# neu-vi/Superpoints_Registration

Measured on AMD Instinct MI355X. Metric: point-cloud pairs/sec (16 384 pts/cloud), higher is better.
Workload: dtype f32 (matrix products: range-scaled split-f16x2 MFMA, f32 accumulate; attention weights below 2^-5 of their row sum carried in one f16 plane); 1 GPU; synthetic 16384-pt pairs, full KPConv backbone + superpoint attn + Sinkhorn-SVD pose (3dmatch config, BASELINE configs[1]); streams_per_gpu=1, points_per_cloud=16384, generator=box, point_order=reference, upsample_indices=True, cross_step_overlap=True, streams_inside_a_forward=3: main path, pyramid searches, ResNet shortcut branches

## Files before the change

### include/spr.h

```cpp
#ifndef SPR_H_
#define SPR_H_

#include <stddef.h>
#include <stdint.h>

#ifdef __cplusplus
extern "C" {
#endif

#define SPR_VERSION 6

#define SPR_ACT_NONE 0
#define SPR_ACT_RELU 1
#define SPR_ACT_SIGMOID 2

#define SPR_ORDER_REFERENCE 0
#define SPR_ORDER_CANONICAL 1

#define SPR_SELECT_NEAREST 0
#define SPR_SELECT_INDEX 1

int spr_version(void);
const char* spr_last_error(void);

// ... 75 lines not shown
                      int k, unsigned int* rkeys, unsigned int* extra, float* noise, unsigned int* skeys, void* stream);
size_t spr_modelnet_pairs_workspace_size(int n_total, int nb, int k);
int spr_modelnet_pairs(const float* xyz, const int* cu, int n_total, int nb, int max_len_host, float p_src, float p_tgt,
                       double q_src, double q_tgt, int k, float scale, float clip, const float* transform,
                       const double* dirs, uint64_t seed, const uint64_t* pair_key, const unsigned int* rkeys,
                       const unsigned int* extra, const float* noise, const unsigned int* skeys, float* src_xyz,
                       float* tgt_xyz, float* pose, unsigned char* src_overlap, unsigned char* tgt_overlap,
                       int* src_index, int* tgt_index, int* corr, int* corr_count, int* status, void* ws,
                       size_t ws_bytes, void* stream);

size_t spr_kpconv_workspace_bytes(int nq, int ns, int cin, int cout);
size_t spr_kpconv_plan_bytes(int nq);
int spr_kpconv_plan(const int* nbr, int nq, int ns, int nbr_stride, int kmax, int rows_sorted,
                    const int* order, void* plan, size_t plan_bytes, void* stream);
size_t spr_kpconv_wplanes_bytes(int cin, int cout);
int spr_kpconv_prep_weights(const float* weights, int n_kp, int cin, int cout, const float* w_range,
                            int w_range_n, void* wplanes, size_t wplanes_bytes, void* stream);
int spr_kpconv_fwd(const float* q_xyz, int nq, const float* s_xyz, int ns, const int* nbr,
                   int nbr_stride, int kmax, int rows_sorted, const float* x, int cin,
                   const float* weights, int cout, const float* kernel_points, int n_kp,
                   float kp_extent, float* out, int impl, const float* x_range, int x_range_n,
                   const float* w_range, int w_range_n, const void* plan, const void* wplanes,
                   void* ws, size_t ws_bytes, void* stream);

size_t spr_instnorm_workspace_bytes(int max_len_host, int nb, int c);
int spr_instnorm(const float* x, const int* cu, int n, int nb, int max_len_host, int c,
                 float eps, int norm, const float* add, float slope, float* out,
                 float* out_range, int out_range_n, void* ws, size_t ws_bytes, void* stream);
int spr_instnorm_stats(const float* x, const int* cu, int n, int nb, int max_len_host, int c, float eps,
                       float* mean, float* rstd, void* ws, size_t ws_bytes, void* stream);

int spr_block_tail_tile_rows(int ka, int kb, int n_out);
size_t spr_block_tail_tiles_len(int n, int nb, int tile_rows);
int spr_block_tail_tiles(const int* cu, int n, int nb, int tile_rows, int* tiles, void* stream);
size_t spr_block_tail_workspace_bytes(int n, int nb, int kb, int n_out, int tile_rows);
int spr_block_tail(const float* xa, int ka, const float* wa, const float* xb, int kb, const float* wb,
                   const float* add, const int* cu, const int* tiles, int n, int nb, int n_out, float eps,
                   float slope, float* out, const float* xa_range, int xa_range_n, const float* wa_range,
                   int wa_range_n, const float* xb_range, int xb_range_n, const float* wb_range,
                   int wb_range_n, float* out_range, int out_range_n, const float* xa_mean,
                   const float* xa_rstd, float xa_slope, void* ws, size_t ws_bytes, void* stream);

int spr_maxpool_gather(const float* x, int ns, int c, const int* idx, int nq, int idx_stride, int k,
                       const int* order, float* out, float* out_range, int out_range_n, void* stream);
size_t spr_cell_order_workspace_bytes(int n);
int spr_cell_order(const float* xyz, const int* cu, int n, int nb, float cell, int* order, void* ws, size_t ws_bytes,
// ... 242 lines not shown
```

### superpoints_registration_amd/_lib.py

```python
import ctypes
import os
import subprocess

_HERE = os.path.dirname(os.path.abspath(__file__))
LIB_PATH = os.environ.get("SPR_HIP_LIB") or os.path.join(_HERE, "libspr_hip.so")

_vp = ctypes.c_void_p
_i = ctypes.c_int
_f = ctypes.c_float
_sz = ctypes.c_size_t
_l = ctypes.c_long
_u64 = ctypes.c_uint64
_d = ctypes.c_double

SIGNATURES = {
    "spr_version": (_i, []),
    "spr_last_error": (ctypes.c_char_p, []),
    "spr_grid_subsample_workspace_bytes": (_sz, [_i, _i]),
    "spr_grid_subsample": (_i, [_vp, _vp, _i, _i, _f, _i, _i, _vp, _vp, _vp, _vp, _sz, _vp]),
    "spr_voxel_downsample_workspace_bytes": (_sz, [_i]),
    "spr_voxel_downsample": (_i, [_vp, _i, ctypes.c_double, _vp, _vp, _vp, _sz, _vp]),
    "spr_prepare_scans_scratch_len": (_sz, [_i, _i]),
    "spr_prepare_scans": (_i, [_vp, _i, _vp, _i, _i, ctypes.c_double, ctypes.c_double, _i, _vp, _sz, _vp, _vp, _vp, _vp,
                               _vp]),
# ... 8 lines not shown
    "spr_radius_table_count": (_i, [_vp, _vp, _i, _i, _i, _i, _f, _vp, _vp, _vp, _i, _vp, _vp]),
    "spr_kdtree_replay_size": (_sz, [_i, _i]),
    "spr_kdtree_replay_build": (_i, [_vp, _vp, _i, _i, _vp, _sz, _vp]),
    "spr_tie_order_workspace_size": (_sz, [_i, _i, _i]),
    "spr_tie_order": (_i, [_vp, _vp, _i, _vp, _vp, _i, _i, _f, _vp, _i, _vp, _i, _i, _i, _vp, _vp, _sz, _vp]),
    "spr_tie_order_host": (_i, [_vp, _vp, _i, _vp, _vp, _i, _i, _f, _vp, _i, _i, _i, _vp]),
    "spr_std_sort_replay_host": (_i, [_vp, _i, _vp, _vp]),
    "spr_gt_overlap_workspace_bytes": (_sz, [_i, _i, _i]),
    "spr_gt_overlap": (_i, [_vp, _vp, _i, _vp, _vp, _i, _vp, _i, ctypes.c_double, _vp, _vp, _vp, _vp, _vp, _vp, _vp,
                            _sz, _vp]),
    "spr_philox4x32_host": (_i, [_vp, _vp, _vp]),
    "spr_augment_draw": (_i, [_u64, _vp, _i, _i, _vp, _vp, _vp, _vp, _vp, _i, _vp, _i, _vp, _vp, _vp]),
    "spr_augment_workspace_bytes": (_sz, [_i, _i, _i, _i]),
    "spr_augment_pairs": (_i, [_vp, _vp, _i, _vp, _vp, _i, _vp, _i, _vp, _vp, _vp, _i, _vp, _vp, _vp, _vp, _i, _f, _i,
                               _u64, _vp, _vp, _vp, _vp, _vp, _vp, _vp, _vp, _vp, _vp, _vp, _vp, _vp, _vp, _vp, _vp,
                               _sz, _vp]),
    "spr_modelnet_draw": (_i, [_u64, _vp, _i, _d, _d, _vp, _vp, _vp, _vp, _i, _i, _vp, _vp, _vp, _vp, _vp]),
    "spr_modelnet_pairs_workspace_size": (_sz, [_i, _i, _i]),
    "spr_modelnet_pairs": (_i, [_vp, _vp, _i, _i, _i, _f, _f, _d, _d, _i, _f, _f, _vp, _vp, _u64, _vp, _vp, _vp, _vp,
                                _vp, _vp, _vp, _vp, _vp, _vp, _vp, _vp, _vp, _vp, _vp, _vp, _sz, _vp]),
    "spr_kpconv_workspace_bytes": (_sz, [_i, _i, _i, _i]),
    "spr_kpconv_fwd": (_i, [_vp, _i, _vp, _i, _vp, _i, _i, _i, _vp, _i, _vp, _i, _vp, _i, _f, _vp, _i, _vp, _i, _vp,
                            _i, _vp, _vp, _vp, _sz, _vp]),
    "spr_instnorm_workspace_bytes": (_sz, [_i, _i, _i]),
    "spr_instnorm": (_i, [_vp, _vp, _i, _i, _i, _i, _f, _i, _vp, _f, _vp, _vp, _i, _vp, _sz, _vp]),
    "spr_maxpool_gather": (_i, [_vp, _i, _i, _vp, _i, _i, _i, _vp, _vp, _vp, _i, _vp]),
    "spr_linear_workspace_bytes": (_sz, []),
    "spr_linear": (_i, [_vp, _i, _i, _vp, _i, _vp, _vp, _i, _vp, _vp, _i, _vp, _i, _vp, _i, _vp, _vp, _sz, _vp]),
    "spr_range_parts": (_i, []),
    "spr_absmax_multi": (_i, [_vp, _i, _i, _vp, _vp]),
    "spr_absmax": (_i, [_vp, _l, _i, _l, _vp, _vp]),
    "spr_kpconv_plan_bytes": (_sz, [_i]),
    "spr_kpconv_plan": (_i, [_vp, _i, _i, _i, _i, _i, _vp, _vp, _sz, _vp]),
    "spr_kpconv_wplanes_bytes": (_sz, [_i, _i]),
    "spr_kpconv_prep_weights": (_i, [_vp, _i, _i, _i, _vp, _i, _vp, _sz, _vp]),
    "spr_block_tail_tile_rows": (_i, [_i, _i, _i]),
    "spr_block_tail_tiles_len": (_sz, [_i, _i, _i]),
    "spr_block_tail_tiles": (_i, [_vp, _i, _i, _i, _vp, _vp]),
    "spr_block_tail_workspace_bytes": (_sz, [_i, _i, _i, _i, _i]),
    "spr_block_tail": (_i, [_vp, _i, _vp, _vp, _i, _vp, _vp, _vp, _vp, _i, _i, _i, _f, _f, _vp, _vp, _i, _vp, _i,
                            _vp, _i, _vp, _i, _vp, _i, _vp, _vp, _f, _vp, _sz, _vp]),
    "spr_instnorm_stats": (_i, [_vp, _vp, _i, _i, _i, _i, _f, _vp, _vp, _vp, _sz, _vp]),
    "spr_cell_order_workspace_bytes": (_sz, [_i]),
    "spr_cell_order": (_i, [_vp, _vp, _i, _i, _f, _vp, _vp, _sz, _vp]),
    "spr_layernorm_range_count": (_i, [_i]),
    "spr_attn_inproj_prepare": (_i, [_vp, _i, _vp, _vp]),
# ... 124 lines not shown
```

### superpoints_registration_amd/csrc/kpconv.hip

```cpp
#include "lds_dma.h"
#include "spr_common.h"
#include "split_mma.h"

namespace spr {
namespace {

constexpr int kKP = 15;

__global__ __launch_bounds__(256) void k_rowflag(const float* __restrict__ x, const float* __restrict__ s_xyz,
                                                 int ns, int cin, unsigned char* __restrict__ flag,
                                                 float4* __restrict__ sxf, int* __restrict__ tile_ctr) {
  const int wid = (blockIdx.x * blockDim.x + threadIdx.x) >> 6;
  const int lane = threadIdx.x & 63;
  const int c4 = cin >> 2;
  if (blockIdx.x == 0 && threadIdx.x == 0) {
    sxf[ns] = make_float4(-1.0e17f, -1.0e17f, -1.0e17f, __int_as_float(0));
    tile_ctr[0] = 0;
  }
  if ((cin & 3) == 0 && c4 <= 64 && (c4 & (c4 - 1)) == 0) {
    constexpr int kRfSteps = 4;
    const int rpl = 64 / c4;
    const int sub = lane / c4, chunk = lane % c4;
    const int row0 = wid * rpl * kRfSteps + sub;
    float4 v[kRfSteps];
// ... 64 lines not shown
    cnt += flag[idx];
    const float rx = s_xyz[3 * (size_t)idx] - qx, ry = s_xyz[3 * (size_t)idx + 1] - qy,
                rz = s_xyz[3 * (size_t)idx + 2] - qz;
    for (int p = 0; p < n_kp; ++p) {
      const float dx = rx - kpts[3 * p], dy = ry - kpts[3 * p + 1], dz = rz - kpts[3 * p + 2];
      const float w = fmaxf(0.f, 1.f - sqrtf(dx * dx + dy * dy + dz * dz) * inv_extent);
      if (w > 0.f) {
        float d = 0.f;
        for (int c = 0; c < cin; ++c)
          d += x[(size_t)idx * cin + c] * W[((size_t)p * cin + c) * cout + o];
        acc += w * d;
      }
    }
  }
  out[(size_t)n * cout + o] = acc / (float)max(cnt, 1);
}

__global__ __launch_bounds__(256) void k_records_cin1(const float* __restrict__ x, const float* __restrict__ s_xyz,
                                                      int ns, float4* __restrict__ sxf) {
  const int i = blockIdx.x * blockDim.x + threadIdx.x;
  if (i < ns) sxf[i] = make_float4(s_xyz[3 * (size_t)i], s_xyz[3 * (size_t)i + 1], s_xyz[3 * (size_t)i + 2], x[i]);
}

__global__ __launch_bounds__(256) void k_kpconv_cin1(
    const float* __restrict__ q_xyz, int nq, const float* __restrict__ s_xyz, int ns,
    const int* __restrict__ nbr, int nbr_stride, int kmax, int rows_sorted,
    const float4* __restrict__ sxf, const float* __restrict__ W, int cout,
    const float* __restrict__ kpts, int n_kp, float inv_extent, float* __restrict__ out) {
  const int lane = threadIdx.x & 63, wave = threadIdx.x >> 6;
  const int qv = lane & 15, g = lane >> 4;
  const int q0 = blockIdx.x * 64 + wave * 16;
  if (q0 >= nq) return;
  const int n = min(q0 + qv, nq - 1);
  const float qx = q_xyz[3 * (size_t)n], qy = q_xyz[3 * (size_t)n + 1], qz = q_xyz[3 * (size_t)n + 2];
  float kx[4], ky[4], kz[4];
  bool kok[4];
#pragma unroll
  for (int s = 0; s < 4; ++s) {
    const int p = 4 * s + g;
    kok[s] = p < n_kp;
    kx[s] = kok[s] ? kpts[3 * p] : 0.f;
    ky[s] = kok[s] ? kpts[3 * p + 1] : 0.f;
    kz[s] = kok[s] ? kpts[3 * p + 2] : 0.f;
  }
  float wf[4] = {0.f, 0.f, 0.f, 0.f};
  int cnt = 0;
  const int* row = nbr + (size_t)n * nbr_stride;
  for (int k = 0; k < kmax; ++k) {
    const int idx = row[k];
    const bool ok = idx >= 0 && idx < ns;
    if (rows_sorted && __ballot(ok) == 0ull) break;
    const size_t id = ok ? (size_t)idx : 0;
    const float4 rec = sxf[id];
    const float xv = ok ? rec.w : 0.f;
    cnt += xv > 0.f ? 1 : 0;
    const float rx = rec.x - qx, ry = rec.y - qy, rz = rec.z - qz;
#pragma unroll
    for (int s = 0; s < 4; ++s) {
      const float dx = rx - kx[s], dy = ry - ky[s], dz = rz - kz[s];
      const float w = fmaxf(0.f, 1.f - __builtin_amdgcn_sqrtf(dx * dx + dy * dy + dz * dz) * inv_extent);
      wf[s] += kok[s] ? w * xv : 0.f;
    }
  }
  const float inv = 1.f / (float)max(cnt, 1);
#pragma unroll
  for (int s = 0; s < 4; ++s) wf[s] *= inv;
  for (int o0 = 0; o0 < cout; o0 += 16) {
    f32x4 acc = {0.f, 0.f, 0.f, 0.f};
#pragma unroll
    for (int s = 0; s < 4; ++s) {
      const int p = 4 * s + g;
      const float bv = (p < n_kp && o0 + qv < cout) ? W[(size_t)p * cout + o0 + qv] : 0.f;
      acc = __builtin_amdgcn_mfma_f32_16x16x4f32(wf[s], bv, acc, 0, 0, 0);
    }
#pragma unroll
    for (int r = 0; r < 4; ++r) {
      const int qn = q0 + 4 * g + r;
      if (qn < nq && o0 + qv < cout) out[(size_t)qn * cout + o0 + qv] = acc[r];
    }
  }
}

__global__ __launch_bounds__(256) void k_w_prep(const float* __restrict__ W, int cin, int cout, int cc,
                                                const float* __restrict__ w_parts, int n_wparts,
                                                _Float16* __restrict__ Wh, _Float16* __restrict__ Wl) {
  __shared__ float sh[17];
  const float sb = pow2f(pow2_exp_for(block_absmax(w_parts, sh, n_wparts)));
  const int total = kKP * cin * cout;
  const int i = blockIdx.x * blockDim.x + threadIdx.x;
  if (i >= total) return;
  const int KS = kKP * cc / 32, NT = cout / 16;
  const int e = i & 7, lane = (i >> 3) & 63;
  int r = i >> 9;
  const int ks = r % KS;
  r /= KS;
  const int nt = r % NT, chunk = r / NT;
  const int p16 = lane & 15, j4 = lane >> 4;
  const int kk = 32 * ks + 8 * j4 + e;
  const int p = kk / cc, c = chunk * cc + kk % cc;
  const float w = W[((size_t)p * cin + c) * cout + 16 * nt + p16] * sb;
  const _Float16 h = (_Float16)w;
  Wh[i] = h;
  Wl[i] = (_Float16)(w - (float)h);
// ... 843 lines not shown
extern "C" size_t spr_kpconv_wplanes_bytes(int cin, int cout) {
  return measure(wplanes_view, cin, cout);
}

extern "C" int spr_kpconv_prep_weights(const float* weights, int n_kp, int cin, int cout, const float* w_range,
                                       int w_range_n, void* wplanes, size_t bytes, void* stream_) {
  hipStream_t stream = (hipStream_t)stream_;
  SPR_REQUIRE(n_kp == kKP && cin % 32 == 0 && cout % 32 == 0 && cout <= 256,
              "kpconv weight planes exist for the MFMA shapes only (15 kernel points, channels in multiples of 32)");
  SPR_REQUIRE(w_range != nullptr && w_range_n >= 1, "kpconv weight planes: the weight range is required");
  Workspace w(wplanes, bytes);
  const auto [wh, wl] = wplanes_view(w, cin, cout);
  SPR_REQUIRE(wplanes != nullptr && w.ok(), "kpconv weight planes: buffer too small");
  hipLaunchKernelGGL(k_w_prep, dim3(cdiv((long)n_kp * cin * cout, 256)), dim3(256), 0, stream, weights, cin, cout,
                     w_chunk(cin), w_range, w_range_n, wh, wl);
  SPR_LAUNCH_CHECK();
  return 0;
}

extern "C" size_t spr_kpconv_workspace_bytes(int nq, int ns, int cin, int cout) {
  return measure(kpconv_layout, nq, ns, cin, cout);
}

extern "C" int spr_kpconv_fwd(const float* q_xyz, int nq, const float* s_xyz, int ns,
                              const int* nbr, int nbr_stride, int kmax, int rows_sorted,
                              const float* x, int cin, const float* weights, int cout,
                              const float* kernel_points, int n_kp, float kp_extent,
                              float* out, int impl, const float* x_range, int x_range_n, const float* w_range,
                              int w_range_n, const void* plan, const void* wplanes, void* ws, size_t ws_bytes,
                              void* stream_) {
  hipStream_t stream = (hipStream_t)stream_;
  SPR_REQUIRE((x_range == nullptr || x_range_n >= 1) && (w_range == nullptr || w_range_n >= 1),
              "kpconv: a range needs a count");
  SPR_REQUIRE(nq > 0 && ns > 0, "kpconv: empty input");
  SPR_REQUIRE(kmax >= 1 && kmax <= nbr_stride, "kpconv: bad kmax=%d stride=%d", kmax, nbr_stride);
  SPR_REQUIRE(cin >= 1 && cout >= 1 && n_kp >= 1 && n_kp <= 32, "kpconv: bad dims");
  SPR_REQUIRE(kp_extent > 0.f, "kpconv: KP_extent must be > 0");
  Workspace w(ws, ws_bytes);
  const auto [flag, sxf, own_wplanes, x_parts, w_parts, own_plan, tile_ctr] = kpconv_layout(w, nq, ns, cin, cout);
  SPR_REQUIRE(ws != nullptr && w.ok(), "kpconv: workspace too small");
  SPR_REQUIRE(wplanes == nullptr || w_range != nullptr, "kpconv: prepared weight planes come with the range they were scaled by");
  Workspace given_w(const_cast<void*>(wplanes), SIZE_MAX), given_p(const_cast<void*>(plan), SIZE_MAX);
  const auto [wh, wl] = wplanes != nullptr ? wplanes_view(given_w, cin, cout) : own_wplanes;
  const float inv_extent = 1.0f / kp_extent;

  if (cin == 1 && (impl == 0 || impl == 2) && n_kp <= 16) {
// ... 66 lines not shown
```

### superpoints_registration_amd/csrc/linear.hip

```cpp
#include <atomic>

#include "attn_planes.h"
#include "lds_dma.h"
#include "spr_common.h"
#include "split_mma.h"

namespace spr {
namespace {

constexpr int BK = 32;
static_assert(BK == kPlaneK, "the split kernels stage split_mma.h's slabs");
constexpr int LDSK = BK + 1;

template <int ACT, bool RES>
__device__ __forceinline__ float store_tile(const f32x16& acc, int row0, int col, int M, int N,
                                            float bv, const float* __restrict__ residual,
                                            float* __restrict__ out, int lh, float unscale = 1.0f,
                                            const float* __restrict__ epi = nullptr) {
  if (col >= N) return 0.f;
  float vmax = 0.f;
  float res[16];
  if (RES) {
#pragma unroll
    for (int r = 0; r < 16; ++r) {
// ... 588 lines not shown
      *reinterpret_cast<float4*>(out_pos + o) = yp;
    }
  }
  if (range_norm || range_pos) {
    mxn = wave_max(mxn);
    mxp = wave_max(mxp);
    if (lane == 0) {
      shr[threadIdx.x >> 6] = mxn;
      shr[4 + (threadIdx.x >> 6)] = mxp;
    }
    __syncthreads();
    if (threadIdx.x == 0) {
      const int slot = blockIdx.x & (kLnRangeSlots - 1);
      if (range_norm)
        atomicMax(reinterpret_cast<unsigned int*>(range_norm) + slot,
                  __float_as_uint(fmaxf(fmaxf(shr[0], shr[1]), fmaxf(shr[2], shr[3]))));
      if (range_pos)
        atomicMax(reinterpret_cast<unsigned int*>(range_pos) + slot,
                  __float_as_uint(fmaxf(fmaxf(shr[4], shr[5]), fmaxf(shr[6], shr[7]))));
    }
  }
}

__global__ void k_posemb(const float* __restrict__ xyz, int n, int d_model, int npf, float scale,
                         float temperature, float* __restrict__ out) {
  const long gid = (long)blockIdx.x * blockDim.x + threadIdx.x;
  if (gid >= (long)n * d_model) return;
  const int row = (int)(gid / d_model), ch = (int)(gid % d_model);
  float v = 0.f;
  if (ch < 3 * npf) {
    const int axis = ch / npf, i = ch % npf;
    const float e = (float)(2 * (i / 2)) / (float)npf;
    const float dim_t = powf(temperature, e);
    const float a = (xyz[3 * (size_t)row + axis] * scale) / dim_t;
    v = (i & 1) ? cosf(a) : sinf(a);
  }
  out[gid] = v;
}

}
}

using namespace spr;

namespace {
template <int ACT, bool RES>
int launch_gemm(const float* x, int m, int k, const float* w, int n, const float* bias,
                const float* residual, float* out, const float* a_parts, int n_aparts, const float* w_parts,
                int n_wparts, float* out_parts, int out_cap, int* out_n, hipStream_t stream) {
  if (out_n) *out_n = 0;
  if (spr::g_gemm_mode.load(std::memory_order_relaxed) == 1) {
    SPR_REQUIRE(a_parts != nullptr && w_parts != nullptr, "linear: split-fp16 mode needs the absmax partials");
    auto lds = [](int bm, int bn) { return (size_t)(bm + bn) * spr::kPlaneStride * 2 * sizeof(_Float16); };
    if (!RES && ACT <= SPR_ACT_SIGMOID && n >= 256 && k == 256 && m >= 1024 && m < 32768) {
      auto kern = spr::k_gemm_nt_h3p<ACT>;
      if (int rc = ensure_dyn_lds((const void*)kern, (int)lds(128, 256))) return rc;
      const int ntiles = cdiv(n, 256) * cdiv(m, 128);
      int grid = device_cu_count();
      grid = grid < ntiles ? grid : ntiles;
      if (grid >= 8) grid &= ~7;
// ... 190 lines not shown
                             float* range_pos, void* stream_) {
  hipStream_t stream = (hipStream_t)stream_;
  SPR_REQUIRE(m > 0 && c % 64 == 0 && c <= 1024, "layernorm: c must be a multiple of 64 and <= 1024 (c=%d)", c);
  SPR_REQUIRE(out_pos == nullptr || pos != nullptr, "layernorm: out_pos needs pos");
  const int grid = cdiv((long)m * 64, 256);
  if (c == 256)
    hipLaunchKernelGGL(k_layernorm256, dim3(cdiv((long)cdiv(m, kLnRows) * 64, 256)), dim3(256), 0, stream, x, m, gamma, beta, eps, pos, out_norm,
                       out_pos, range_norm, range_pos);
  else if (c <= 256)
    hipLaunchKernelGGL(k_layernorm<4>, dim3(grid), dim3(256), 0, stream, x, m, c, gamma, beta, eps,
                       pos, out_norm, out_pos, range_norm, range_pos);
  else
    hipLaunchKernelGGL(k_layernorm<16>, dim3(grid), dim3(256), 0, stream, x, m, c, gamma, beta, eps,
                       pos, out_norm, out_pos, range_norm, range_pos);
  SPR_LAUNCH_CHECK();
  return 0;
}

extern "C" int spr_posemb_sine(const float* xyz, int n, int d_model, float scale, float temperature,
                               float* out, void* stream_) {
  hipStream_t stream = (hipStream_t)stream_;
  SPR_REQUIRE(n > 0 && d_model >= 6, "posemb: bad sizes");
  const int npf = d_model / 3 / 2 * 2;
  const long total = (long)n * d_model;
  hipLaunchKernelGGL(k_posemb, dim3(cdiv(total, 256)), dim3(256), 0, stream, xyz, n, d_model, npf,
                     scale, temperature, out);
  SPR_LAUNCH_CHECK();
  return 0;
}
```

### superpoints_registration_amd/csrc/norm_pool.hip

```cpp
#include "spr_common.h"

namespace spr {
namespace {

constexpr int kSliceRows = 512;
int in_nsplit(int max_len) {
  int s = cdiv(max_len > 0 ? max_len : 1, kSliceRows);
  return s < 1 ? 1 : s;
}

__global__ __launch_bounds__(256) void k_in_stats(const float* __restrict__ x,
                                                  const int* __restrict__ cu, int c, int nsplit,
                                                  double* __restrict__ part ) {
  const int cloud = blockIdx.x, split = blockIdx.y, cb = blockIdx.z * 64;
  const int beg = cu[cloud], end = cu[cloud + 1];
  const int r0 = beg + split * kSliceRows;
  const int r1 = min(r0 + kSliceRows, end);
  const int cw = min(c - cb, 64);
  const int cw4 = cw >> 2;
  const int rl = 256 / cw4;
  const int tc = threadIdx.x % cw4, tr = threadIdx.x / cw4;
  __shared__ double sh[8][256];
  double s[4] = {0, 0, 0, 0}, ss[4] = {0, 0, 0, 0};
  if (tr < rl) {
// ... 42 lines not shown
    }
  }
}

__global__ void k_in_final(const double* __restrict__ part, const int* __restrict__ cu, int nb,
                           int c, int nsplit, float eps, float* __restrict__ mean,
                           float* __restrict__ rstd) {
  const int i = blockIdx.x * blockDim.x + threadIdx.x;
  if (i >= nb * c) return;
  const int cloud = i / c, ch = i % c;
  double s = 0.0, ss = 0.0;
  for (int k = 0; k < nsplit; ++k) {
    const double* p = part + (((size_t)cloud * nsplit + k) * 2) * c;
    s += p[ch];
    ss += p[c + ch];
  }
  const int len = cu[cloud + 1] - cu[cloud];
  const double n = len > 0 ? (double)len : 1.0;
  const double m = s / n;
  double var = ss / n - m * m;
  if (var < 0.0) var = 0.0;
  mean[i] = (float)m;
  rstd[i] = (float)(1.0 / sqrt(var + (double)eps));
}

__device__ __forceinline__ void publish_range(float mx, float* __restrict__ slots, int nslots) {
  __shared__ float shr[4];
  mx = wave_max(mx);
  if ((threadIdx.x & 63) == 0) shr[threadIdx.x >> 6] = mx;
  __syncthreads();
  if (threadIdx.x == 0)
    atomicMax(reinterpret_cast<unsigned int*>(slots) + (blockIdx.x & (nslots - 1)),
              __float_as_uint(fmaxf(fmaxf(shr[0], shr[1]), fmaxf(shr[2], shr[3]))));
}

constexpr int kInApplyUnroll = 4;
__global__ __launch_bounds__(256) void k_in_apply(const float* __restrict__ x, const int* __restrict__ cu, int n,
                                                  int nb, int c, int norm, const float* __restrict__ mean,
                                                  const float* __restrict__ rstd, const float* __restrict__ add,
                                                  float slope, float* __restrict__ out,
                                                  float* __restrict__ out_range, int nslots) {
  const int c4 = c >> 2;
  const long total = (long)n * c4;
  const long stride = (long)gridDim.x * blockDim.x;
  const long g0 = (long)blockIdx.x * blockDim.x + threadIdx.x;
  float4 v[kInApplyUnroll], a[kInApplyUnroll];
#pragma unroll
  for (int u = 0; u < kInApplyUnroll; ++u) {
    const long gid = g0 + u * stride;
    if (gid < total) {
      v[u] = reinterpret_cast<const float4*>(x)[gid];
      if (add) a[u] = reinterpret_cast<const float4*>(add)[gid];
    }
  }
  float mx = 0.f;
#pragma unroll
// ... 184 lines not shown
    float4 v = make_float4(0.f, 0.f, 0.f, 0.f);
    if (id >= 0 && id < ns) v = reinterpret_cast<const float4*>(x + (size_t)id * c)[q];
    m.x = fmaxf(m.x, v.x);
    m.y = fmaxf(m.y, v.y);
    m.z = fmaxf(m.z, v.z);
    m.w = fmaxf(m.w, v.w);
  }
  reinterpret_cast<float4*>(out)[gid] = m;
  mx = fmaxf(fmaxf(fabsf(m.x), fabsf(m.y)), fmaxf(fabsf(m.z), fabsf(m.w)));
  }
  if (out_range != nullptr) publish_range(mx, out_range, nslots);
}

__global__ void k_gather_rows(const float* __restrict__ x, int n_src, int c,
                              const int* __restrict__ idx, int n, float* __restrict__ out) {
  const long gid = (long)blockIdx.x * blockDim.x + threadIdx.x;
  if (gid >= (long)n * c) return;
  const int row = (int)(gid / c), ch = (int)(gid % c);
  const int id = idx[row];
  out[gid] = (id >= 0 && id < n_src) ? x[(size_t)id * c + ch] : 0.f;
}

}
}

using namespace spr;

namespace {
struct InstnormWs {
  double* part;
  float *mean, *rstd;
  double *m1, *m2;
};
InstnormWs instnorm_layout(Workspace& w, int max_len, int nb, int c, bool backward) {
  const size_t B = (size_t)(nb > 0 ? nb : 1), C = (size_t)(c > 0 ? c : 1);
  InstnormWs l{};
  l.part = w.take<double>(B * in_nsplit(max_len) * 2 * C);
  l.mean = w.take<float>(B * C);
  l.rstd = w.take<float>(B * C);
  if (backward) {
    l.m1 = w.take<double>(B * C);
    l.m2 = w.take<double>(B * C);
  }
  return l;
}
}
// ... 115 lines not shown
```

### superpoints_registration_amd/csrc/spr_common.h

```cpp
#pragma once
#include <hip/hip_runtime.h>

#include <cstdarg>
#include <cstdio>
#include <cstdint>
#include <cstring>

#include "../../include/spr.h"

namespace spr {

constexpr int kWave = 64;

void set_error(const char* fmt, ...);

#define SPR_HIP_CHECK(expr)                                                   \
  do {                                                                        \
    hipError_t _e = (expr);                                                   \
    if (_e != hipSuccess) {                                                   \
      ::spr::set_error("%s failed: %s (%s:%d)", #expr, hipGetErrorString(_e), \
                       __FILE__, __LINE__);                                   \
      return 1;                                                               \
    }                                                                         \
  } while (0)
// ... 60 lines not shown
  int code, n;
  ProfScope(hipStream_t s, int code_, int n_) : stream(s), on(prof_enabled()), code(code_), n(n_) {
    if (!on) return;
    if (hipEventCreate(&beg) != hipSuccess || hipEventCreate(&end) != hipSuccess) {
      on = false;
      return;
    }
    (void)hipEventRecord(beg, stream);
  }
  ~ProfScope() {
    if (!on) return;
    (void)hipEventRecord(end, stream);
    prof_push(beg, end, code, n);
  }
};

int ensure_dyn_lds(const void* kernel, int bytes);
int device_cu_count();

int launch_absmax(const float* x, long rows, int cols, long stride, float* parts, hipStream_t stream);
int launch_absmax2(const float* x0, long rows0, int cols0, long stride0, float* parts0, const float* x1,
                   long rows1, int cols1, long stride1, float* parts1, hipStream_t stream);

#ifdef __HIPCC__
typedef float f32x2 __attribute__((ext_vector_type(2)));
typedef float f32x4 __attribute__((ext_vector_type(4)));
typedef float f32x16 __attribute__((ext_vector_type(16)));
typedef _Float16 f16x2 __attribute__((ext_vector_type(2)));

__device__ __forceinline__ int find_segment(const int* __restrict__ cu, int nseg,
                                            int i) {
  int lo = 0, hi = nseg;
  while (hi - lo > 1) {
    int mid = (lo + hi) >> 1;
    if (cu[mid] <= i)
      lo = mid;
    else
      hi = mid;
  }
  return lo;
}

__device__ __forceinline__ int xcd_swizzle(int b, int nwg) {
  const int q = nwg >> 3, r = nwg & 7;
  const int xcd = b & 7, idx = b >> 3;
  const int base = (xcd < r) ? xcd * (q + 1) : r * (q + 1) + (xcd - r) * q;
// ... 81 lines not shown
#pragma unroll
  for (int o = 32; o > 0; o >>= 1) v += __shfl_xor(v, o, 64);
  return v;
}
__device__ __forceinline__ double wave_sum_d(double v) {
#pragma unroll
  for (int o = 32; o > 0; o >>= 1) v += __shfl_xor(v, o, 64);
  return v;
}
__device__ __forceinline__ double block_sum_d(double v, double* sh) {
  v = wave_sum_d(v);
  if ((threadIdx.x & 63) == 0) sh[threadIdx.x >> 6] = v;
  __syncthreads();
  double t = 0.0;
  for (int i = 0; i < (int)(blockDim.x >> 6); ++i) t += sh[i];
  __syncthreads();
  return t;
}
__device__ __forceinline__ float wave_max(float v) {
#pragma unroll
  for (int o = 32; o > 0; o >>= 1) v = fmaxf(v, __shfl_xor(v, o, 64));
  return v;
}
#endif

}
```

### superpoints_registration_amd/kpconv_blocks.py

```python
import math

import torch
import torch.nn as nn
from torch.nn.init import kaiming_uniform_
from torch.nn.parameter import Parameter

from . import _concurrency, ops
from .kernel_points import load_kernels


def _cu_of(batch, layer_ind):
    cache = batch.setdefault('_cu', {})
    cu = cache.get(layer_ind)
    if cu is None:
        cu = ops.lengths_to_cu(batch['stack_lengths'][layer_ind],
                               batch['points'][layer_ind].device)
        cache[layer_ind] = cu
    return cu


def _maxlen_of(batch, layer_ind):
    lens = batch.get('_lens_host')
    return max(lens[layer_ind]) if lens is not None else None


def _idx_of(batch, key, layer_ind):
    cache = batch.setdefault('_i32', {})
    t = cache.get((key, layer_ind))
    if t is None:
        t = batch[key][layer_ind].to(torch.int32)
# ... 143 lines not shown
        self.block_name = block_name
        self.in_dim = in_dim
        self.out_dim = out_dim
        self.KPConv = KPConv(config.num_kernel_points, config.in_points_dim, in_dim, out_dim // 2,
                             current_extent, radius,
                             fixed_kernel_points=config.fixed_kernel_points,
                             KP_influence=config.KP_influence,
                             aggregation_mode=config.aggregation_mode,
                             deformable='deform' in block_name, modulated=config.modulated)
        self.batch_norm = BatchNormBlock(out_dim // 2, self.use_bn, self.bn_momentum)
        self.leaky_relu = nn.LeakyReLU(0.1)

    def forward(self, x, batch):
        li = self.layer_ind
        if 'strided' in self.block_name:
            q_pts, s_pts = batch['points'][li + 1], batch['points'][li]
            neighb_inds = _idx_of(batch, 'pools', li)
            stack_lengths, cu, ml = batch['stack_lengths'][li + 1], _cu_of(batch, li + 1), _maxlen_of(batch, li + 1)
        else:
            q_pts = s_pts = batch['points'][li]
            neighb_inds = _idx_of(batch, 'neighbors', li)
            stack_lengths, cu, ml = batch['stack_lengths'][li], _cu_of(batch, li), _maxlen_of(batch, li)
        self.KPConv.rows_sorted = bool(batch.get('_rows_sorted', False))
        x = self.KPConv(q_pts, s_pts, neighb_inds, x)
        return self.batch_norm(x, stack_lengths, cu=cu, slope=0.1, max_len=ml)


class ResnetBottleneckBlock(nn.Module):

    def __init__(self, block_name, in_dim, out_dim, radius, layer_ind, config):
        super().__init__()
        current_extent = radius * config.KP_extent / config.conv_radius
        self.bn_momentum = config.batch_norm_momentum
        self.use_bn = config.use_batch_norm
        self.block_name = block_name
        self.layer_ind = layer_ind
        self.in_dim = in_dim
        self.out_dim = out_dim
        if in_dim != out_dim // 4:
            self.unary1 = UnaryBlock(in_dim, out_dim // 4, self.use_bn, self.bn_momentum)
        else:
            self.unary1 = nn.Identity()
        self.KPConv = KPConv(config.num_kernel_points, config.in_points_dim, out_dim // 4,
                             out_dim // 4, current_extent, radius,
                             fixed_kernel_points=config.fixed_kernel_points,
                             KP_influence=config.KP_influence,
# ... 91 lines not shown
```

Baseline: 1281 pairs/s.

## Fuse cin=1 KPConv stem with instance norm via low-rank kernel-weight sums

```diff
diff --git a/include/spr.h b/include/spr.h
--- a/include/spr.h
+++ b/include/spr.h
@@ -121,6 +121,14 @@
                    float kp_extent, float* out, int impl, const float* x_range, int x_range_n,
                    const float* w_range, int w_range_n, const void* plan, const void* wplanes,
                    void* ws, size_t ws_bytes, void* stream);
+
+int spr_kpconv_stem_supported(int cin, int cout, int n_kp);
+size_t spr_kpconv_stem_workspace_size(int nq, int ns, int nb, int max_len_host, int cout);
+int spr_kpconv_stem(const float* q_xyz, int nq, const float* s_xyz, int ns, const int* nbr, int nbr_stride,
+                    int kmax, int rows_sorted, const float* x, const float* weights, int cout,
+                    const float* kernel_points, int n_kp, float kp_extent, const int* cu, int nb,
+                    int max_len_host, float eps, float slope, float* out, float* out_range, int out_range_n,
+                    float* mean_out, float* rstd_out, void* ws, size_t ws_bytes, void* stream);
 
 size_t spr_instnorm_workspace_bytes(int max_len_host, int nb, int c);
 int spr_instnorm(const float* x, const int* cu, int n, int nb, int max_len_host, int c,
diff --git a/superpoints_registration_amd/_lib.py b/superpoints_registration_amd/_lib.py
--- a/superpoints_registration_amd/_lib.py
+++ b/superpoints_registration_amd/_lib.py
@@ -54,6 +54,10 @@
     "spr_kpconv_workspace_bytes": (_sz, [_i, _i, _i, _i]),
     "spr_kpconv_fwd": (_i, [_vp, _i, _vp, _i, _vp, _i, _i, _i, _vp, _i, _vp, _i, _vp, _i, _f, _vp, _i, _vp, _i, _vp,
                             _i, _vp, _vp, _vp, _sz, _vp]),
+    "spr_kpconv_stem_supported": (_i, [_i, _i, _i]),
+    "spr_kpconv_stem_workspace_size": (_sz, [_i, _i, _i, _i, _i]),
+    "spr_kpconv_stem": (_i, [_vp, _i, _vp, _i, _vp, _i, _i, _i, _vp, _vp, _i, _vp, _i, _f, _vp, _i, _i, _f, _f, _vp,
+                             _vp, _i, _vp, _vp, _vp, _sz, _vp]),
     "spr_instnorm_workspace_bytes": (_sz, [_i, _i, _i]),
     "spr_instnorm": (_i, [_vp, _vp, _i, _i, _i, _i, _f, _i, _vp, _f, _vp, _vp, _i, _vp, _sz, _vp]),
     "spr_maxpool_gather": (_i, [_vp, _i, _i, _vp, _i, _i, _i, _vp, _vp, _vp, _i, _vp]),
diff --git a/superpoints_registration_amd/csrc/kpconv.hip b/superpoints_registration_amd/csrc/kpconv.hip
--- a/superpoints_registration_amd/csrc/kpconv.hip
+++ b/superpoints_registration_amd/csrc/kpconv.hip
@@ -110,15 +110,20 @@
   if (i < ns) sxf[i] = make_float4(s_xyz[3 * (size_t)i], s_xyz[3 * (size_t)i + 1], s_xyz[3 * (size_t)i + 2], x[i]);
 }
 
-__global__ __launch_bounds__(256) void k_kpconv_cin1(
-    const float* __restrict__ q_xyz, int nq, const float* __restrict__ s_xyz, int ns,
-    const int* __restrict__ nbr, int nbr_stride, int kmax, int rows_sorted,
-    const float4* __restrict__ sxf, const float* __restrict__ W, int cout,
-    const float* __restrict__ kpts, int n_kp, float inv_extent, float* __restrict__ out) {
+constexpr int kCin1Chunk = 64;
+constexpr int kCin1RowStride = kCin1Chunk + 1;
+constexpr int kCin1Batch = 8;
+constexpr int kCin1LdsInts = 4 * 16 * kCin1RowStride + 32;
+
+template <int B>
+__device__ __forceinline__ void cin1_gather(const float* __restrict__ q_xyz, int nq, int ns,
+                                            const int* __restrict__ nbr, int nbr_stride, int kmax, int rows_sorted,
+                                            const float4* __restrict__ sxf, const float* __restrict__ kpts, int n_kp,
+                                            float inv_extent, int* __restrict__ lrows, float (&wf)[4]) {
+  static_assert(B >= 1 && B <= 32, "the last batch's reads past the last staged row stay inside the slack");
   const int lane = threadIdx.x & 63, wave = threadIdx.x >> 6;
   const int qv = lane & 15, g = lane >> 4;
   const int q0 = blockIdx.x * 64 + wave * 16;
-  if (q0 >= nq) return;
   const int n = min(q0 + qv, nq - 1);
   const float qx = q_xyz[3 * (size_t)n], qy = q_xyz[3 * (size_t)n + 1], qz = q_xyz[3 * (size_t)n + 2];
   float kx[4], ky[4], kz[4];
@@ -131,28 +136,86 @@
     ky[s] = kok[s] ? kpts[3 * p + 1] : 0.f;
     kz[s] = kok[s] ? kpts[3 * p + 2] : 0.f;
   }
-  float wf[4] = {0.f, 0.f, 0.f, 0.f};
+#pragma unroll
+  for (int s = 0; s < 4; ++s) wf[s] = 0.f;
   int cnt = 0;
-  const int* row = nbr + (size_t)n * nbr_stride;
-  for (int k = 0; k < kmax; ++k) {
-    const int idx = row[k];
-    const bool ok = idx >= 0 && idx < ns;
-    if (rows_sorted && __ballot(ok) == 0ull) break;
-    const size_t id = ok ? (size_t)idx : 0;
-    const float4 rec = sxf[id];
-    const float xv = ok ? rec.w : 0.f;
-    cnt += xv > 0.f ? 1 : 0;
-    const float rx = rec.x - qx, ry = rec.y - qy, rz = rec.z - qz;
-#pragma unroll
-    for (int s = 0; s < 4; ++s) {
-      const float dx = rx - kx[s], dy = ry - ky[s], dz = rz - kz[s];
-      const float w = fmaxf(0.f, 1.f - __builtin_amdgcn_sqrtf(dx * dx + dy * dy + dz * dz) * inv_extent);
-      wf[s] += kok[s] ? w * xv : 0.f;
+  int* lrow = lrows + wave * 16 * kCin1RowStride;
+  bool done = q0 >= nq;
+  for (int c0 = 0; c0 < kmax; c0 += kCin1Chunk) {
+    const int kc = min(kCin1Chunk, kmax - c0);
+    if (c0 > 0) __syncthreads();
+    {
+      int v[4][kCin1Chunk / 16];
+#pragma unroll
+      for (int i = 0; i < 4; ++i) {
+        const int* src = nbr + (size_t)min(q0 + g + 4 * i, nq - 1) * nbr_stride + c0;
+#pragma unroll
+        for (int j = 0; j < kCin1Chunk / 16; ++j) {
+          const int c = qv + 16 * j;
+          v[i][j] = (!done && c < kc) ? src[c] : -1;
+        }
+      }
+#pragma unroll
+      for (int i = 0; i < 4; ++i)
+#pragma unroll
+        for (int j = 0; j < kCin1Chunk / 16; ++j) lrow[(g + 4 * i) * kCin1RowStride + qv + 16 * j] = v[i][j];
+    }
+    __syncthreads();
+    if (done) continue;
+    int kstop = kc;
+    if (rows_sorted) {
+      int first = kc;
+      for (int k = g; k < kc; k += 4) {
+        const int idx = lrow[qv * kCin1RowStride + k];
+        if (!(idx >= 0 && idx < ns)) first = min(first, k);
+      }
+      first = min(first, __shfl_xor(first, 16, 64));
+      first = min(first, __shfl_xor(first, 32, 64));
+#pragma unroll
+      for (int o = 8; o > 0; o >>= 1) first = max(first, __shfl_xor(first, o, 64));
+      kstop = first;
+      done = kstop < kc;
+    }
+    for (int k0 = 0; k0 < kstop; k0 += B) {
+      float4 rec[B];
+      bool ok[B];
+#pragma unroll
+      for (int b = 0; b < B; ++b) {
+        const int idx = lrow[qv * kCin1RowStride + k0 + b];
+        ok[b] = k0 + b < kstop && idx >= 0 && idx < ns;
+        rec[b] = sxf[ok[b] ? (size_t)idx : 0];
+      }
+#pragma unroll
+      for (int b = 0; b < B; ++b) {
+        const float xv = ok[b] ? rec[b].w : 0.f;
+        cnt += xv > 0.f ? 1 : 0;
+        const float rx = rec[b].x - qx, ry = rec[b].y - qy, rz = rec[b].z - qz;
+#pragma unroll
+        for (int s = 0; s < 4; ++s) {
+          const float dx = rx - kx[s], dy = ry - ky[s], dz = rz - kz[s];
+          const float w = fmaxf(0.f, 1.f - __builtin_amdgcn_sqrtf(dx * dx + dy * dy + dz * dz) * inv_extent);
+          wf[s] += kok[s] ? w * xv : 0.f;
+        }
+      }
     }
   }
   const float inv = 1.f / (float)max(cnt, 1);
 #pragma unroll
   for (int s = 0; s < 4; ++s) wf[s] *= inv;
+}
+
+__global__ __launch_bounds__(256, 5) void k_kpconv_cin1(
+    const float* __restrict__ q_xyz, int nq, const float* __restrict__ s_xyz, int ns,
+    const int* __restrict__ nbr, int nbr_stride, int kmax, int rows_sorted,
+    const float4* __restrict__ sxf, const float* __restrict__ W, int cout,
+    const float* __restrict__ kpts, int n_kp, float inv_extent, float* __restrict__ out) {
+  __shared__ int lrows[kCin1LdsInts];
+  const int lane = threadIdx.x & 63, wave = threadIdx.x >> 6;
+  const int qv = lane & 15, g = lane >> 4;
+  const int q0 = blockIdx.x * 64 + wave * 16;
+  float wf[4];
+  cin1_gather<kCin1Batch>(q_xyz, nq, ns, nbr, nbr_stride, kmax, rows_sorted, sxf, kpts, n_kp, inv_extent, lrows, wf);
+  if (q0 >= nq) return;
   for (int o0 = 0; o0 < cout; o0 += 16) {
     f32x4 acc = {0.f, 0.f, 0.f, 0.f};
 #pragma unroll
@@ -167,6 +230,116 @@
       if (qn < nq && o0 + qv < cout) out[(size_t)qn * cout + o0 + qv] = acc[r];
     }
   }
+}
+
+constexpr int kStemSliceRows = 512;
+
+__global__ __launch_bounds__(256, 5) void k_stem_sums(
+    const float* __restrict__ q_xyz, int nq, int ns, const int* __restrict__ nbr, int nbr_stride, int kmax,
+    int rows_sorted, const float4* __restrict__ sxf, const float* __restrict__ kpts, int n_kp, float inv_extent,
+    float* __restrict__ S ) {
+  __shared__ int lrows[kCin1LdsInts];
+  const int lane = threadIdx.x & 63, wave = threadIdx.x >> 6;
+  const int qv = lane & 15, g = lane >> 4;
+  const int q = blockIdx.x * 64 + wave * 16 + qv;
+  float wf[4];
+  cin1_gather<kCin1Batch>(q_xyz, nq, ns, nbr, nbr_stride, kmax, rows_sorted, sxf, kpts, n_kp, inv_extent, lrows, wf);
+  if (q >= nq) return;
+#pragma unroll
+  for (int s = 0; s < 4; ++s) S[(size_t)q * 16 + 4 * s + g] = wf[s];
+}
+
+__device__ __forceinline__ void stem_load_group(const float* __restrict__ S, int row0, int end, int qv, int g,
+                                                float (&a)[4]) {
+  const int row = row0 + qv;
+#pragma unroll
+  for (int s = 0; s < 4; ++s) a[s] = row < end ? S[(size_t)row * 16 + 4 * s + g] : 0.f;
+}
+
+__global__ __launch_bounds__(256) void k_stem_stats(const float* __restrict__ S, const int* __restrict__ cu,
+                                                    const float* __restrict__ W, int cout, int n_kp, int nsplit,
+                                                    double* __restrict__ part ) {
+  constexpr int kGroups = kStemSliceRows / 16 / 4;
+  const int cloud = blockIdx.x, split = blockIdx.y;
+  const int lane = threadIdx.x & 63, wave = threadIdx.x >> 6;
+  const int qv = lane & 15, g = lane >> 4;
+  const int end = cu[cloud + 1];
+  const int r0 = cu[cloud] + split * kStemSliceRows;
+  __shared__ double red[2][4][4][16];
+  float a[kGroups][4];
+#pragma unroll
+  for (int i = 0; i < kGroups; ++i) stem_load_group(S, r0 + (wave + 4 * i) * 16, end, qv, g, a[i]);
+  double* p = part + (((size_t)cloud * nsplit + split) * 2) * cout;
+  for (int o0 = 0; o0 < cout; o0 += 16) {
+    float bv[4];
+#pragma unroll
+    for (int s = 0; s < 4; ++s) bv[s] = 4 * s + g < n_kp ? W[(size_t)(4 * s + g) * cout + o0 + qv] : 0.f;
+    double sm = 0.0, sq = 0.0;
+#pragma unroll
+    for (int i = 0; i < kGroups; ++i) {
+      f32x4 acc = {0.f, 0.f, 0.f, 0.f};
+#pragma unroll
+      for (int s = 0; s < 4; ++s) acc = __builtin_amdgcn_mfma_f32_16x16x4f32(a[i][s], bv[s], acc, 0, 0, 0);
+#pragma unroll
+      for (int r = 0; r < 4; ++r) {
+        const double y = acc[r];
+        sm += y;
+        sq += y * y;
+      }
+    }
+    red[0][wave][g][qv] = sm;
+    red[1][wave][g][qv] = sq;
+    __syncthreads();
+    if (threadIdx.x < 32) {
+      const int which = threadIdx.x >> 4, ch = threadIdx.x & 15;
+      double t = 0.0;
+      for (int w = 0; w < 4; ++w)
+        for (int gg = 0; gg < 4; ++gg) t += red[which][w][gg][ch];
+      p[(size_t)which * cout + o0 + ch] = t;
+    }
+    __syncthreads();
+  }
+}
+
+__global__ __launch_bounds__(256) void k_stem_apply(const float* __restrict__ S, int nq, const int* __restrict__ cu,
+                                                    int nb, const float* __restrict__ W, int cout, int n_kp,
+                                                    const float* __restrict__ mean, const float* __restrict__ rstd,
+                                                    float slope, float* __restrict__ out,
+                                                    float* __restrict__ out_range, int nslots) {
+  const int lane = threadIdx.x & 63, wave = threadIdx.x >> 6;
+  const int qv = lane & 15, g = lane >> 4;
+  const int q0 = blockIdx.x * 64 + wave * 16;
+  const int q = q0 + qv;
+  float mx = 0.f;
+  if (q0 < nq) {
+    float b[4];
+    stem_load_group(S, q0, nq, qv, g, b);
+    const int cloud = find_segment(cu, nb, min(q, nq - 1));
+    for (int o0 = 0; o0 < cout; o0 += 16) {
+      f32x4 acc = {0.f, 0.f, 0.f, 0.f};
+#pragma unroll
+      for (int s = 0; s < 4; ++s) {
+        const float av = 4 * s + g < n_kp ? W[(size_t)(4 * s + g) * cout + o0 + qv] : 0.f;
+        acc = __builtin_amdgcn_mfma_f32_16x16x4f32(av, b[s], acc, 0, 0, 0);
+      }
+      if (q < nq) {
+        const float4 m = *reinterpret_cast<const float4*>(mean + (size_t)cloud * cout + o0 + 4 * g);
+        const float4 r = *reinterpret_cast<const float4*>(rstd + (size_t)cloud * cout + o0 + 4 * g);
+        float4 w;
+        w.x = (acc[0] - m.x) * r.x;
+        w.y = (acc[1] - m.y) * r.y;
+        w.z = (acc[2] - m.z) * r.z;
+        w.w = (acc[3] - m.w) * r.w;
+        w.x = w.x >= 0.f ? w.x : w.x * slope;
+        w.y = w.y >= 0.f ? w.y : w.y * slope;
+        w.z = w.z >= 0.f ? w.z : w.z * slope;
+        w.w = w.w >= 0.f ? w.w : w.w * slope;
+        *reinterpret_cast<float4*>(out + (size_t)q * cout + o0 + 4 * g) = w;
+        mx = fmaxf(mx, fmaxf(fmaxf(fabsf(w.x), fabsf(w.y)), fmaxf(fabsf(w.z), fabsf(w.w))));
+      }
+    }
+  }
+  if (out_range != nullptr) publish_range(mx, out_range, nslots);
 }
 
 __global__ __launch_bounds__(256) void k_w_prep(const float* __restrict__ W, int cin, int cout, int cc,
@@ -1056,6 +1229,71 @@
   return measure(kpconv_layout, nq, ns, cin, cout);
 }
 
+namespace {
+struct StemWs {
+  float4* sxf;
+  float* S;
+  double* part;
+  float *mean, *rstd;
+};
+StemWs stem_layout(Workspace& w, int nq, int ns, int nb, int max_len, int cout) {
+  const size_t Q = (size_t)(nq > 0 ? nq : 1), N = (size_t)(ns > 0 ? ns : 1), B = (size_t)(nb > 0 ? nb : 1),
+               C = (size_t)(cout > 0 ? cout : 1);
+  StemWs l{};
+  l.sxf = w.take<float4>(N);
+  l.S = w.take<float>(Q * 16);
+  l.part = w.take<double>(B * instnorm_nsplit(max_len) * 2 * C);
+  l.mean = w.take<float>(B * C);
+  l.rstd = w.take<float>(B * C);
+  return l;
+}
+}
+
+extern "C" int spr_kpconv_stem_supported(int cin, int cout, int n_kp) {
+  return cin == 1 && cout >= 16 && cout % 16 == 0 && n_kp >= 1 && n_kp <= 16;
+}
+
+extern "C" size_t spr_kpconv_stem_workspace_size(int nq, int ns, int nb, int max_len, int cout) {
+  return measure(stem_layout, nq, ns, nb, max_len, cout);
+}
+
+extern "C" int spr_kpconv_stem(const float* q_xyz, int nq, const float* s_xyz, int ns, const int* nbr, int nbr_stride,
+                               int kmax, int rows_sorted, const float* x, const float* weights, int cout,
+                               const float* kernel_points, int n_kp, float kp_extent, const int* cu, int nb,
+                               int max_len_host, float eps, float slope, float* out, float* out_range,
+                               int out_range_n, float* mean_out, float* rstd_out, void* ws, size_t ws_bytes,
+                               void* stream_) {
+  hipStream_t stream = (hipStream_t)stream_;
+  SPR_REQUIRE(nq > 0 && ns > 0 && nb >= 1, "kpconv_stem: empty input");
+  SPR_REQUIRE(kmax >= 1 && kmax <= nbr_stride, "kpconv_stem: bad kmax=%d stride=%d", kmax, nbr_stride);
+  SPR_REQUIRE(spr_kpconv_stem_supported(1, cout, n_kp), "kpconv_stem: no kernel for cout=%d, %d kernel points", cout,
+              n_kp);
+  SPR_REQUIRE(kp_extent > 0.f, "kpconv_stem: KP_extent must be > 0");
+  SPR_REQUIRE(max_len_host >= 1 && max_len_host <= nq, "kpconv_stem: bad max_len_host=%d", max_len_host);
+  SPR_REQUIRE(out_range == nullptr || (out_range_n >= 1 && (out_range_n & (out_range_n - 1)) == 0),
+              "kpconv_stem: out_range_n must be a power of two");
+  SPR_REQUIRE(instnorm_slice_rows() == kStemSliceRows, "kpconv_stem: statistics slices differ from the InstanceNorm's");
+  Workspace w(ws, ws_bytes);
+  const StemWs l = stem_layout(w, nq, ns, nb, max_len_host, cout);
+  SPR_REQUIRE(ws != nullptr && w.ok(), "kpconv_stem: workspace too small");
+  const int nsplit = instnorm_nsplit(max_len_host);
+  float* mean = mean_out != nullptr ? mean_out : l.mean;
+  float* rstd = rstd_out != nullptr ? rstd_out : l.rstd;
+  hipLaunchKernelGGL(k_records_cin1, dim3(cdiv(ns, 256)), dim3(256), 0, stream, x, s_xyz, ns, l.sxf);
+  {
+    ProfScope prof(stream, 100000 + cout, nq);
+    hipLaunchKernelGGL(k_stem_sums, dim3(cdiv(nq, 64)), dim3(256), 0, stream, q_xyz, nq, ns, nbr, nbr_stride, kmax,
+                       rows_sorted, l.sxf, kernel_points, n_kp, 1.0f / kp_extent, l.S);
+  }
+  hipLaunchKernelGGL(k_stem_stats, dim3(nb, nsplit), dim3(256), 0, stream, l.S, cu, weights, cout, n_kp, nsplit,
+                     l.part);
+  launch_in_final(l.part, cu, nb, cout, nsplit, eps, mean, rstd, stream);
+  hipLaunchKernelGGL(k_stem_apply, dim3(cdiv(nq, 64)), dim3(256), 0, stream, l.S, nq, cu, nb, weights, cout, n_kp,
+                     mean, rstd, slope, out, out_range, out_range_n);
+  SPR_LAUNCH_CHECK();
+  return 0;
+}
+
 extern "C" int spr_kpconv_fwd(const float* q_xyz, int nq, const float* s_xyz, int ns,
                               const int* nbr, int nbr_stride, int kmax, int rows_sorted,
                               const float* x, int cin, const float* weights, int cout,
diff --git a/superpoints_registration_amd/csrc/linear.hip b/superpoints_registration_amd/csrc/linear.hip
--- a/superpoints_registration_amd/csrc/linear.hip
+++ b/superpoints_registration_amd/csrc/linear.hip
@@ -634,20 +634,43 @@
   }
 }
 
-__global__ void k_posemb(const float* __restrict__ xyz, int n, int d_model, int npf, float scale,
-                         float temperature, float* __restrict__ out) {
-  const long gid = (long)blockIdx.x * blockDim.x + threadIdx.x;
-  if (gid >= (long)n * d_model) return;
-  const int row = (int)(gid / d_model), ch = (int)(gid % d_model);
-  float v = 0.f;
-  if (ch < 3 * npf) {
-    const int axis = ch / npf, i = ch % npf;
-    const float e = (float)(2 * (i / 2)) / (float)npf;
-    const float dim_t = powf(temperature, e);
-    const float a = (xyz[3 * (size_t)row + axis] * scale) / dim_t;
-    v = (i & 1) ? cosf(a) : sinf(a);
-  }
-  out[gid] = v;
+constexpr int kPosembTokens = 16;
+constexpr int kPosembMaxFreq = 1024;
+
+__global__ __launch_bounds__(256) void k_posemb(const float* __restrict__ xyz, int n, int d_model, int npf,
+                                                float scale, float temperature, float* __restrict__ out) {
+  __shared__ float dim_t[kPosembMaxFreq];
+  for (int f = threadIdx.x; f < npf / 2; f += 256) dim_t[f] = powf(temperature, (float)(2 * f) / (float)npf);
+  __syncthreads();
+  const int slots = (d_model + 1) >> 1;
+  const bool vec = (d_model & 1) == 0;
+  const int row0 = blockIdx.x * kPosembTokens;
+  const int rows = min(kPosembTokens, n - row0);
+  const int dr = 256 / slots, ds = 256 % slots;
+  int r = (int)threadIdx.x / slots, s = (int)threadIdx.x % slots;
+  while (r < rows) {
+    const int row = row0 + r, ch = 2 * s;
+    float v0 = 0.f, v1 = 0.f;
+    if (ch < 3 * npf) {
+      const int axis = (ch >= npf ? 1 : 0) + (ch >= 2 * npf ? 1 : 0), i = ch - axis * npf;
+      const float a = (xyz[3 * (size_t)row + axis] * scale) / dim_t[i >> 1];
+      v0 = sinf(a);
+      v1 = cosf(a);
+    }
+    float* o = out + (size_t)row * d_model + ch;
+    if (vec) {
+      *reinterpret_cast<float2*>(o) = make_float2(v0, v1);
+    } else {
+      o[0] = v0;
+      if (ch + 1 < d_model) o[1] = v1;
+    }
+    s += ds;
+    r += dr;
+    if (s >= slots) {
+      s -= slots;
+      ++r;
+    }
+  }
 }
 
 }
@@ -884,8 +907,8 @@
   hipStream_t stream = (hipStream_t)stream_;
   SPR_REQUIRE(n > 0 && d_model >= 6, "posemb: bad sizes");
   const int npf = d_model / 3 / 2 * 2;
-  const long total = (long)n * d_model;
-  hipLaunchKernelGGL(k_posemb, dim3(cdiv(total, 256)), dim3(256), 0, stream, xyz, n, d_model, npf,
+  SPR_REQUIRE(npf / 2 <= kPosembMaxFreq, "posemb: d_model=%d is wider than the frequency table", d_model);
+  hipLaunchKernelGGL(k_posemb, dim3(cdiv(n, kPosembTokens)), dim3(256), 0, stream, xyz, n, d_model, npf,
                      scale, temperature, out);
   SPR_LAUNCH_CHECK();
   return 0;
diff --git a/superpoints_registration_amd/csrc/norm_pool.hip b/superpoints_registration_amd/csrc/norm_pool.hip
--- a/superpoints_registration_amd/csrc/norm_pool.hip
+++ b/superpoints_registration_amd/csrc/norm_pool.hip
@@ -88,16 +88,6 @@
   if (var < 0.0) var = 0.0;
   mean[i] = (float)m;
   rstd[i] = (float)(1.0 / sqrt(var + (double)eps));
-}
-
-__device__ __forceinline__ void publish_range(float mx, float* __restrict__ slots, int nslots) {
-  __shared__ float shr[4];
-  mx = wave_max(mx);
-  if ((threadIdx.x & 63) == 0) shr[threadIdx.x >> 6] = mx;
-  __syncthreads();
-  if (threadIdx.x == 0)
-    atomicMax(reinterpret_cast<unsigned int*>(slots) + (blockIdx.x & (nslots - 1)),
-              __float_as_uint(fmaxf(fmaxf(shr[0], shr[1]), fmaxf(shr[2], shr[3]))));
 }
 
 constexpr int kInApplyUnroll = 4;
@@ -328,6 +318,14 @@
 }
 
 }
+
+int instnorm_slice_rows() { return kSliceRows; }
+int instnorm_nsplit(int max_len) { return in_nsplit(max_len); }
+void launch_in_final(const double* part, const int* cu, int nb, int c, int nsplit, float eps, float* mean,
+                     float* rstd, hipStream_t stream) {
+  hipLaunchKernelGGL(k_in_final, dim3(cdiv((long)nb * c, 256)), dim3(256), 0, stream, part, cu, nb, c, nsplit, eps,
+                     mean, rstd);
+}
 }
 
 using namespace spr;
diff --git a/superpoints_registration_amd/csrc/spr_common.h b/superpoints_registration_amd/csrc/spr_common.h
--- a/superpoints_registration_amd/csrc/spr_common.h
+++ b/superpoints_registration_amd/csrc/spr_common.h
@@ -106,6 +106,11 @@
 int launch_absmax2(const float* x0, long rows0, int cols0, long stride0, float* parts0, const float* x1,
                    long rows1, int cols1, long stride1, float* parts1, hipStream_t stream);
 
+int instnorm_slice_rows();
+int instnorm_nsplit(int max_len);
+void launch_in_final(const double* part, const int* cu, int nb, int c, int nsplit, float eps, float* mean,
+                     float* rstd, hipStream_t stream);
+
 #ifdef __HIPCC__
 typedef float f32x2 __attribute__((ext_vector_type(2)));
 typedef float f32x4 __attribute__((ext_vector_type(4)));
@@ -233,6 +238,15 @@
   for (int o = 32; o > 0; o >>= 1) v = fmaxf(v, __shfl_xor(v, o, 64));
   return v;
 }
+__device__ __forceinline__ void publish_range(float mx, float* __restrict__ slots, int nslots) {
+  __shared__ float shr[4];
+  mx = wave_max(mx);
+  if ((threadIdx.x & 63) == 0) shr[threadIdx.x >> 6] = mx;
+  __syncthreads();
+  if (threadIdx.x == 0)
+    atomicMax(reinterpret_cast<unsigned int*>(slots) + (blockIdx.x & (nslots - 1)),
+              __float_as_uint(fmaxf(fmaxf(shr[0], shr[1]), fmaxf(shr[2], shr[3]))));
+}
 #endif
 
 }
diff --git a/superpoints_registration_amd/kpconv_blocks.py b/superpoints_registration_amd/kpconv_blocks.py
--- a/superpoints_registration_amd/kpconv_blocks.py
+++ b/superpoints_registration_amd/kpconv_blocks.py
@@ -5,7 +5,7 @@
 from torch.nn.init import kaiming_uniform_
 from torch.nn.parameter import Parameter
 
-from . import _concurrency, ops
+from . import _concurrency, ops, stem
 from .kernel_points import load_kernels
 
 
@@ -195,6 +195,11 @@
             neighb_inds = _idx_of(batch, 'neighbors', li)
             stack_lengths, cu, ml = batch['stack_lengths'][li], _cu_of(batch, li), _maxlen_of(batch, li)
         self.KPConv.rows_sorted = bool(batch.get('_rows_sorted', False))
+        if stem.stem_route(x, self.KPConv.weights, self.use_bn):
+            return stem.kpconv_stem(q_pts, s_pts, neighb_inds, x, self.KPConv.weights,
+                                    self.KPConv.kernel_points.detach(), self.KPConv.KP_extent, cu,
+                                    eps=self.batch_norm.eps, slope=0.1, rows_sorted=self.KPConv.rows_sorted,
+                                    max_len=ml)
         x = self.KPConv(q_pts, s_pts, neighb_inds, x)
         return self.batch_norm(x, stack_lengths, cu=cu, slope=0.1, max_len=ml)
 
diff --git a/superpoints_registration_amd/stem.py b/superpoints_registration_amd/stem.py
--- /dev/null
+++ b/superpoints_registration_amd/stem.py
@@ -0,0 +1,61 @@
+from typing import Optional
+
+import torch
+
+from . import _lib, ops
+
+
+def stem_shape_ok(cin: int, cout: int, n_kp: int) -> bool:
+    return cin == 1 and cout >= 16 and cout % 16 == 0 and 1 <= n_kp <= 16
+
+
+def stem_predicate(on_gpu: bool, wants_grad: bool, use_bn: bool, x_channels: int, weights_shape) -> bool:
+    if not on_gpu or wants_grad or not use_bn or len(weights_shape) != 3:
+        return False
+    n_kp, cin, cout = (int(v) for v in weights_shape)
+    return int(x_channels) == cin and stem_shape_ok(cin, cout, n_kp)
+
+
+def stem_route(x, weights, use_bn: bool) -> bool:
+    if not (isinstance(x, torch.Tensor) and x.dim() == 2):
+        return False
+    return stem_predicate(x.is_cuda, ops._wants_grad(x, weights), bool(use_bn), x.shape[1], tuple(weights.shape))
+
+
+def kpconv_stem(q_pts, s_pts, nbr, x, weights, kernel_points, kp_extent: float, cu, eps: float = 1e-5,
+                slope: float = 0.1, rows_sorted: bool = False, max_len: Optional[int] = None,
+                return_stats: bool = False):
+    q_pts = ops._dev(q_pts, "q_pts", torch.float32)
+    s_pts = ops._dev(s_pts, "s_pts", torch.float32)
+    x = ops._dev(x, "x", torch.float32)
+    weights = ops._dev(weights.detach(), "weights", torch.float32)
+    kernel_points = ops._dev(kernel_points, "kernel_points", torch.float32)
+    cu = ops._dev(cu, "cu", torch.int32)
+    if not nbr.is_cuda:
+        raise RuntimeError("neighb_inds must be on the device")
+    if nbr.dtype != torch.int32:
+        nbr = nbr.to(torch.int32)
+    stride = nbr.stride(0) if nbr.stride(1) == 1 and nbr.shape[1] > 0 else None
+    if stride is None:
+        nbr = nbr.contiguous()
+        stride = nbr.shape[1]
+    nq, ns, kmax = q_pts.shape[0], s_pts.shape[0], nbr.shape[1]
+    n_kp, cin, cout = weights.shape
+    if not stem_shape_ok(int(cin), int(cout), int(n_kp)) or x.shape != (ns, 1):
+        raise RuntimeError(f"kpconv_stem: no kernel for x {tuple(x.shape)}, weights {tuple(weights.shape)}")
+    nb = cu.numel() - 1
+    max_len = nq if max_len is None else max(1, min(int(max_len), nq))
+    L = _lib.lib()
+    ws = ops._workspace(L.spr_kpconv_stem_workspace_size(nq, ns, nb, max_len, cout), x.device)
+    out = torch.empty((nq, cout), dtype=torch.float32, device=x.device)
+    cnt = ops._STREAM_SLOTS
+    rng = ops._zero_slots(cnt, x.device)
+    st = torch.empty((2, nb, cout), dtype=torch.float32, device=x.device) if return_stats else None
+    _lib.check(L.spr_kpconv_stem(ops._ptr(q_pts), nq, ops._ptr(s_pts), ns, ops._ptr(nbr), int(stride), kmax,
+                                 int(bool(rows_sorted)), ops._ptr(x), ops._ptr(weights), cout,
+                                 ops._ptr(kernel_points), n_kp, float(kp_extent), ops._ptr(cu), nb, max_len,
+                                 float(eps), float(slope), ops._ptr(out), ops._ptr(rng), cnt,
+                                 ops._ptr(None if st is None else st[0]), ops._ptr(None if st is None else st[1]),
+                                 ops._ptr(ws), ws.numel(), ops._stream(x)), "spr_kpconv_stem")
+    ops._set_range(out, rng, cnt)
+    return (out, st[0], st[1]) if return_stats else out
```

Measured after the change: 1296 pairs/s (median of 6 runs). 1.1% higher.
